# JakobHavtorn/benchmarking-lvms

Measured on AMD Instinct MI355X. Metric: audio frames/sec training (VRNN, 16 kHz mu-law), higher is better.
Workload: dtype f32

## Files before the change

benchmarking-lvms_amd/blvm/_hip.py:

```python
import ctypes
import os

import torch

_LIB_PATH = os.environ.get("BLVM_HIP_LIB") or os.path.join(os.path.dirname(os.path.abspath(__file__)), "lib", "libblvm_hip.so")
_lib = None

c_int, c_float, c_void_p, c_size_t, c_double = ctypes.c_int, ctypes.c_float, ctypes.c_void_p, ctypes.c_size_t, ctypes.c_double


class BlvmHipError(RuntimeError):
    pass


class VrnnWeights(ctypes.Structure):

    _fields_ = [
        ("prior_w", c_void_p * 3), ("prior_b", c_void_p * 3), ("prior_hw", c_void_p), ("prior_hb", c_void_p),
        ("post_w", c_void_p * 3), ("post_b", c_void_p * 3), ("post_hw", c_void_p), ("post_hb", c_void_p),
        ("phi_w", c_void_p * 4), ("phi_b", c_void_p * 4),
        ("gru_wih", c_void_p), ("gru_whh", c_void_p), ("gru_bih", c_void_p), ("gru_bhh", c_void_p),
    ]


class VrnnDecodeWeights(ctypes.Structure):

    _fields_ = [
        ("enc_w", c_void_p * 3), ("enc_b", c_void_p * 3), ("cell", ctypes.POINTER(VrnnWeights)),
        ("dec_w", c_void_p * 3), ("dec_b", c_void_p * 3), ("lik_w", c_void_p), ("lik_b", c_void_p),
    ]


class SrnnWeights(ctypes.Structure):

    _fields_ = [
        ("prior_w", c_void_p * 3), ("prior_b", c_void_p * 3), ("prior_hw", c_void_p), ("prior_hb", c_void_p),
        ("post_w", c_void_p * 3), ("post_b", c_void_p * 3), ("post_hw", c_void_p), ("post_hb", c_void_p),
    ]


class SrnnDecodeWeights(ctypes.Structure):

    _fields_ = [
        ("enc_w", c_void_p * 3), ("enc_b", c_void_p * 3), ("gru_wih", c_void_p), ("gru_whh", c_void_p), ("gru_bih", c_void_p),
        ("gru_bhh", c_void_p), ("chain", ctypes.POINTER(SrnnWeights)), ("dec_w", c_void_p * 3), ("dec_b", c_void_p * 3),
        ("lik_w", c_void_p), ("lik_b", c_void_p),
    ]


class LstmDecodeWeights(ctypes.Structure):

    _fields_ = [
        ("emb_w", c_void_p * 3), ("emb_b", c_void_p * 3), ("wih", ctypes.POINTER(c_void_p)), ("whh", ctypes.POINTER(c_void_p)),
        ("bih", ctypes.POINTER(c_void_p)), ("bhh", ctypes.POINTER(c_void_p)), ("dec_w", c_void_p * 3), ("dec_b", c_void_p * 3),
        ("lik_w", c_void_p), ("lik_b", c_void_p),
    ]


class RssmWeights(ctypes.Structure):

    _fields_ = [
        ("gin_w", c_void_p), ("gin_b", c_void_p), ("gru_wih", c_void_p), ("gru_whh", c_void_p), ("gru_bih", c_void_p),
        ("gru_bhh", c_void_p),
        ("prior_w", c_void_p * 3), ("prior_b", c_void_p * 3), ("prior_hw", c_void_p), ("prior_hb", c_void_p),
        ("post_w", c_void_p * 3), ("post_b", c_void_p * 3), ("post_hw", c_void_p), ("post_hb", c_void_p),
    ]


_SIGNATURES = {
    "blvm_upload_i32": (c_int, [c_void_p, c_int, c_void_p, c_void_p]),
    "blvm_version": (c_int, []),
    "blvm_last_error": (ctypes.c_char_p, []),
    "blvm_device_ok": (c_int, []),
    "blvm_async_errors": (c_int, [c_void_p]),
    "blvm_async_errors_take": (c_int, [c_void_p]),
    "blvm_pchain_configure": (c_int, [c_int, c_int]),
    "blvm_pchain_max_batch": (c_int, []),
    "blvm_set_operand_dtype": (c_int, [c_int]),
    "blvm_get_operand_dtype": (c_int, []),
    "blvm_pchain_profile": (c_int, [c_void_p]),
    "blvm_pchain_tune": (c_int, [c_int]),
    "blvm_pchain_static": (c_int, [c_int]),
    "blvm_rnn_path_counts": (c_int, [c_void_p]),
    "blvm_rssm_path_counts": (c_int, [c_void_p]),
    "blvm_pchain_chain_probe": (c_int, [c_void_p, c_void_p, c_void_p, c_void_p, c_int, c_int, c_int, c_int, c_void_p]),
    "blvm_pchain_static_chain_probe": (c_int, [c_void_p, c_void_p, c_void_p, c_void_p, c_int, c_int, c_int, c_int, c_void_p]),
    "blvm_pchain_static_chain_probe_fetch": (c_int, [c_void_p, c_void_p, c_void_p, c_void_p, c_int, c_int, c_int, c_int, c_void_p]),
    "blvm_pchain_static_chain_probe_paced": (c_int, [c_void_p, c_void_p, c_void_p, c_void_p] + [c_int] * 6 + [c_void_p]),
    "blvm_pchain_rows_to_t16": (c_int, [c_void_p, c_int, c_int, c_int, c_void_p, c_void_p]),
    "blvm_gemm_f32": (c_int, [c_int, c_int, c_int, c_int, c_int, c_void_p, c_int, c_void_p, c_int, c_void_p, c_int,
                              c_void_p, c_int, c_float, c_void_p, c_int, c_int, c_int, c_void_p]),
    "blvm_act_bwd_f32": (c_int, [c_void_p, c_void_p, c_float, c_void_p, c_size_t, c_void_p]),
    "blvm_colsum_f32": (c_int, [c_int, c_int, c_void_p, c_int, c_void_p, c_int, c_void_p]),
    "blvm_wgrad_f32": (c_int, [c_int, c_int, c_int, c_void_p, c_int, c_void_p, c_int, c_void_p, c_int, c_void_p, c_int, c_void_p]),
    "blvm_wgrad_group_f32": (c_int, [c_int, c_void_p, c_void_p, c_int, c_void_p, c_void_p, c_void_p, c_void_p, c_void_p, c_void_p, c_void_p, c_void_p]),
    "blvm_dmol_fwd": (c_int, [c_void_p, c_int, c_void_p, c_void_p, c_void_p, c_void_p, c_int, c_int, c_int, c_int,
                              c_int, c_int, c_float, c_void_p, c_void_p, c_void_p]),
    "blvm_dmol_bwd": (c_int, [c_void_p, c_int, c_void_p, c_void_p, c_void_p, c_void_p, c_void_p, c_int, c_int, c_int,
                              c_int, c_int, c_int, c_float, c_void_p, c_void_p, c_void_p]),
    "blvm_dmol_bwd_fused_workspace_floats": (c_size_t, [c_int] * 3),
    "blvm_dmol_bwd_fused": (c_int, [c_void_p, c_int, c_void_p, c_void_p, c_void_p, c_void_p, c_void_p, c_int, c_int, c_int,
                                    c_int, c_int, c_int, c_float, c_float, c_void_p, c_void_p, c_void_p, c_void_p, c_void_p]),
    "blvm_elbo_fwd": (c_int, [c_void_p, c_void_p, c_void_p, c_double, c_double, c_int, c_int, c_void_p, c_void_p, c_void_p, c_void_p]),
    "blvm_elbo_bwd": (c_int, [c_void_p, c_void_p, c_double, c_double, c_int, c_void_p, c_void_p, c_void_p]),
    "blvm_kl_fwd": (c_int, [c_void_p, c_void_p, c_void_p, c_void_p, c_int, c_void_p, c_int, c_int, c_int, c_int,
                            c_float, c_void_p, c_void_p, c_void_p]),
    "blvm_kl_bwd": (c_int, [c_void_p, c_void_p, c_void_p, c_void_p, c_int, c_void_p, c_void_p, c_void_p, c_int, c_int,
                            c_int, c_int, c_float, c_void_p, c_void_p, c_void_p, c_void_p, c_void_p]),
    "blvm_vrnn_decode_scratch_floats": (c_size_t, [c_int] * 4),
    "blvm_vrnn_decode": (c_int, [ctypes.POINTER(VrnnDecodeWeights)] + [c_void_p] * 5 + [c_int] * 7 + [c_float] * 3 + [c_void_p] * 4),
    "blvm_srnn_generate_scratch_floats": (c_size_t, [c_int] * 6),
    "blvm_srnn_generate": (c_int, [ctypes.POINTER(SrnnDecodeWeights)] + [c_void_p] * 6 + [c_int] * 7 + [c_float] * 3 + [c_void_p] * 5),
    "blvm_lstm_generate_scratch_floats": (c_size_t, [c_int] * 5),
    "blvm_lstm_generate": (c_int, [ctypes.POINTER(LstmDecodeWeights)] + [c_void_p] * 5 + [c_int] * 6 + [c_float] + [c_void_p] * 5),
    "blvm_lstm_generate_any_stack": (c_int, [ctypes.POINTER(LstmDecodeWeights)] + [c_void_p] * 5 + [c_int] * 6 + [c_float] + [c_void_p] * 5),
    "blvm_vrnn_generate_scratch_floats": (c_size_t, [c_int] * 6),
    "blvm_vrnn_generate": (c_int, [ctypes.POINTER(VrnnDecodeWeights)] + [c_void_p] * 5 + [c_int] * 7 + [c_float] * 3 + [c_void_p] * 4),
    "blvm_vrnn_reserve_floats": (c_size_t, [c_int] * 6),
    "blvm_vrnn_bwd_workspace_floats": (c_size_t, [c_int] * 6),
    "blvm_vrnn_seq_fwd": (c_int, [ctypes.POINTER(VrnnWeights), c_void_p, c_void_p, c_void_p, c_int, c_int, c_int, c_int,
                                  c_int, c_int, c_int, c_float, c_void_p, c_void_p, c_void_p, c_void_p, c_void_p,
                                  c_void_p, c_void_p, c_void_p]),
    "blvm_vrnn_seq_bwd": (c_int, [ctypes.POINTER(VrnnWeights), c_void_p, c_void_p, c_void_p, c_void_p, c_void_p,
                                  c_void_p, c_void_p, c_void_p, c_void_p, c_void_p, c_void_p, c_void_p, c_void_p,
                                  c_int, c_float, c_int, c_int, c_int, c_int, c_int, c_int, c_int, c_float, c_void_p,
                                  c_void_p, ctypes.POINTER(VrnnWeights), c_void_p, c_void_p]),
    "blvm_lstm_reserve_floats": (c_size_t, [c_int] * 3),
    "blvm_lstm_bwd_workspace_floats": (c_size_t, [c_int] * 3),
    "blvm_lstm_seq_fwd": (c_int, [c_void_p] * 8 + [c_int] * 4 + [c_void_p] * 5),
    "blvm_lstm_seq_bwd": (c_int, [c_void_p] * 5 + [c_int] * 4 + [c_void_p] * 9),
    "blvm_gru_reserve_floats": (c_size_t, [c_int] * 3),
    "blvm_gru_bwd_workspace_floats": (c_size_t, [c_int] * 3),
    "blvm_gru_seq_fwd": (c_int, [c_void_p] * 5 + [c_int, c_void_p, c_void_p] + [c_int] * 5 + [c_void_p, ctypes.c_longlong, c_int]
                         + [c_void_p] * 3),
    "blvm_gru_seq_bwd": (c_int, [c_void_p] * 3 + [c_int, c_void_p, c_int, c_void_p, c_void_p, ctypes.c_longlong, c_int]
                         + [c_int] * 4 + [c_void_p, c_int, c_int] + [c_void_p] * 7),
    "blvm_srnn_reserve_floats": (c_size_t, [c_int] * 5),
    "blvm_srnn_bwd_workspace_floats": (c_size_t, [c_int] * 5),
    "blvm_srnn_latent_fwd": (c_int, [ctypes.POINTER(SrnnWeights)] + [c_void_p] * 4 + [c_int] * 6 + [c_float, c_float]
                             + [c_void_p] * 7),
    "blvm_srnn_latent_bwd": (c_int, [ctypes.POINTER(SrnnWeights)] + [c_void_p] * 13 + [c_int, c_float] + [c_int] * 6
                             + [c_float, c_float] + [c_void_p] * 3 + [ctypes.POINTER(SrnnWeights), c_void_p, c_void_p]),
    "blvm_scale_act_f32": (c_int, [c_void_p, c_float, c_float, c_void_p, c_size_t, c_void_p]),
    "blvm_conv1d_k2_workspace_floats": (c_size_t, [c_int] * 2),
    "blvm_conv1d_k2_fwd": (c_int, [c_void_p] * 3 + [c_int] * 5 + [c_void_p] * 3),
    "blvm_conv1d_k2_bwd": (c_int, [c_void_p] * 3 + [c_int] * 5 + [c_void_p] * 5),
    "blvm_wavenet_block_reserve_floats": (c_size_t, [c_int] * 4),
    "blvm_wavenet_block_workspace_floats": (c_size_t, [c_int] * 5),
    "blvm_wavenet_block_fwd": (c_int, [c_void_p] * 5 + [c_int] * 6 + [c_float] + [c_void_p] * 5),
    "blvm_wavenet_block_bwd": (c_int, [c_void_p] * 6 + [c_int] * 6 + [c_float] + [c_void_p] * 7),
    "blvm_wavenet_stack_floats": (c_int, [c_int] * 3 + [c_void_p, c_int, c_void_p, c_void_p]),
    "blvm_wavenet_stack_fwd": (c_int, [c_void_p] * 4 + [c_int] * 6 + [c_float] + [c_void_p] * 5),
    "blvm_wavenet_stack_bwd": (c_int, [c_void_p] * 4 + [c_int] * 6 + [c_float] + [c_void_p] * 8),
    "blvm_wavenet_decode_pack_floats": (c_size_t, [c_int] * 4),
    "blvm_wavenet_decode_scratch_floats": (c_size_t, [c_void_p] + [c_int] * 4),
    "blvm_wavenet_decode": (c_int, [c_void_p] * 2 + [c_int] * 7 + [c_float] * 3 + [c_void_p] * 5),
    "blvm_wavenet_decode_ring_offset_floats": (c_size_t, [c_int] * 3),
    "blvm_wavenet_decode_ring_fill": (c_int, [c_void_p] + [c_int] * 5 + [c_void_p] * 2),
    "blvm_wavenet_decode_resume": (c_int, [c_void_p] * 2 + [c_int] * 8 + [c_float] * 3 + [c_void_p] * 7),
    "blvm_stcn_generate_pack_floats": (c_size_t, [c_int] * 4 + [c_void_p] * 2 + [c_int] * 3),
    "blvm_stcn_generate_scratch_floats": (c_size_t, [c_void_p] + [c_int] * 4 + [c_void_p] * 2 + [c_int] * 4),
    "blvm_stcn_generate": (c_int, [c_void_p] * 3 + [c_int] * 2 + [c_void_p] * 2 + [c_int] * 7 + [c_float] * 6 + [c_void_p] * 9),
    "blvm_stcn_generate_ring_offset_floats": (c_size_t, [c_int] * 4 + [c_void_p] * 2 + [c_int] * 3),
    "blvm_stcn_generate_resume": (c_int, [c_void_p] * 3 + [c_int] * 2 + [c_void_p] * 2 + [c_int] * 7 + [c_float] * 6 + [c_void_p] * 8
                                  + [c_int] + [c_void_p] * 3),
    "blvm_rssm_reserve_floats": (c_size_t, [c_int] * 4),
    "blvm_rssm_bwd_workspace_floats": (c_size_t, [c_int] * 4),
    "blvm_rssm_seq_fwd": (c_int, [ctypes.POINTER(RssmWeights)] + [c_void_p] * 5 + [c_int] * 7 + [c_float] + [c_void_p] * 8),
    "blvm_rssm_seq_bwd": (c_int, [ctypes.POINTER(RssmWeights)] + [c_void_p] * 15 + [c_int, c_float] + [c_int] * 7 + [c_float]
                          + [c_void_p] * 4 + [ctypes.POINTER(RssmWeights), c_void_p, c_void_p]),
    "blvm_gmm_fwd": (c_int, [c_void_p, c_int] + [c_void_p] * 4 + [c_int] * 5 + [c_float] * 2 + [c_void_p] * 3),
    "blvm_gmm_bwd": (c_int, [c_void_p, c_int] + [c_void_p] * 5 + [c_int] * 5 + [c_float] * 2 + [c_void_p] * 3),
    "blvm_gauss_head_fwd": (c_int, [c_void_p, c_int] + [c_void_p] * 4 + [c_int] * 4 + [c_float] * 2 + [c_void_p] * 3),
    "blvm_gauss_head_bwd": (c_int, [c_void_p, c_int] + [c_void_p] * 5 + [c_int] * 4 + [c_float] * 2 + [c_void_p] * 3),
# ... 112 lines not shown
```

benchmarking-lvms_amd/csrc/common.h:

```cpp
#pragma once
#include <hip/hip_runtime.h>
#include <limits.h>
#include <stdint.h>
#include <stdio.h>

#include "blvm_hip.h"

namespace blvm {

typedef float f32x4 __attribute__((ext_vector_type(4)));
typedef float f32x16 __attribute__((ext_vector_type(16)));

void set_error(const char* fmt, ...);

#define BLVM_REQUIRE(cond, ...)            \
  do {                                     \
    if (!(cond)) {                         \
      blvm::set_error(__VA_ARGS__);        \
      return BLVM_EINVAL;                  \
    }                                      \
  } while (0)

#define BLVM_CHECK_LAUNCH(what)                                                     \
  do {                                                                              \
// ... 210 lines not shown
}

template <int NW, bool WT16 = false>
__device__ __forceinline__ f32x16 wave_gemm32(const float* __restrict__ A, int lda, int r0, int nrows,
                                               const float* __restrict__ W, int ldw, int c0, int K, int wave, f32x16 acc) {
  constexpr int STEP = NW * 8;
  const int lane = threadIdx.x & 63, li = lane & 31, lh = lane >> 5;
  const bool aok = (r0 + li) < nrows;
  const float* ap = A + (size_t)(aok ? r0 + li : 0) * lda + 4 * lh;
  const float* wp = WT16 ? W + (size_t)(c0 / 16 + (li >> 4)) * ldw * 16 + ((li & 15) + 16 * lh) * 4 : W + (size_t)(c0 + li) * ldw + 4 * lh;
  constexpr int WS = WT16 ? 16 : 1;
  const float4 zero = make_float4(0.f, 0.f, 0.f, 0.f);
  int kc = wave * 8;
  for (; kc + 3 * STEP < K; kc += 4 * STEP) {
    float4 a0 = *reinterpret_cast<const float4*>(ap + kc);
    float4 a1 = *reinterpret_cast<const float4*>(ap + kc + STEP);
    float4 a2 = *reinterpret_cast<const float4*>(ap + kc + 2 * STEP);
    float4 a3 = *reinterpret_cast<const float4*>(ap + kc + 3 * STEP);
    const float4 w0 = *reinterpret_cast<const float4*>(wp + WS * (kc));
    const float4 w1 = *reinterpret_cast<const float4*>(wp + WS * (kc + STEP));
    const float4 w2 = *reinterpret_cast<const float4*>(wp + WS * (kc + 2 * STEP));
    const float4 w3 = *reinterpret_cast<const float4*>(wp + WS * (kc + 3 * STEP));
    if (!aok) { a0 = a1 = a2 = a3 = zero; }
    acc = __builtin_amdgcn_mfma_f32_32x32x2f32(a0.x, w0.x, acc, 0, 0, 0);
    acc = __builtin_amdgcn_mfma_f32_32x32x2f32(a0.y, w0.y, acc, 0, 0, 0);
    acc = __builtin_amdgcn_mfma_f32_32x32x2f32(a0.z, w0.z, acc, 0, 0, 0);
    acc = __builtin_amdgcn_mfma_f32_32x32x2f32(a0.w, w0.w, acc, 0, 0, 0);
    acc = __builtin_amdgcn_mfma_f32_32x32x2f32(a1.x, w1.x, acc, 0, 0, 0);
    acc = __builtin_amdgcn_mfma_f32_32x32x2f32(a1.y, w1.y, acc, 0, 0, 0);
    acc = __builtin_amdgcn_mfma_f32_32x32x2f32(a1.z, w1.z, acc, 0, 0, 0);
    acc = __builtin_amdgcn_mfma_f32_32x32x2f32(a1.w, w1.w, acc, 0, 0, 0);
    acc = __builtin_amdgcn_mfma_f32_32x32x2f32(a2.x, w2.x, acc, 0, 0, 0);
    acc = __builtin_amdgcn_mfma_f32_32x32x2f32(a2.y, w2.y, acc, 0, 0, 0);
    acc = __builtin_amdgcn_mfma_f32_32x32x2f32(a2.z, w2.z, acc, 0, 0, 0);
    acc = __builtin_amdgcn_mfma_f32_32x32x2f32(a2.w, w2.w, acc, 0, 0, 0);
    acc = __builtin_amdgcn_mfma_f32_32x32x2f32(a3.x, w3.x, acc, 0, 0, 0);
    acc = __builtin_amdgcn_mfma_f32_32x32x2f32(a3.y, w3.y, acc, 0, 0, 0);
    acc = __builtin_amdgcn_mfma_f32_32x32x2f32(a3.z, w3.z, acc, 0, 0, 0);
    acc = __builtin_amdgcn_mfma_f32_32x32x2f32(a3.w, w3.w, acc, 0, 0, 0);
  }
  for (; kc < K; kc += STEP) {
    float4 a0 = *reinterpret_cast<const float4*>(ap + kc);
    const float4 w0 = *reinterpret_cast<const float4*>(wp + WS * (kc));
    if (!aok) a0 = zero;
    acc = __builtin_amdgcn_mfma_f32_32x32x2f32(a0.x, w0.x, acc, 0, 0, 0);
    acc = __builtin_amdgcn_mfma_f32_32x32x2f32(a0.y, w0.y, acc, 0, 0, 0);
    acc = __builtin_amdgcn_mfma_f32_32x32x2f32(a0.z, w0.z, acc, 0, 0, 0);
    acc = __builtin_amdgcn_mfma_f32_32x32x2f32(a0.w, w0.w, acc, 0, 0, 0);
  }
  return acc;
}

template <int G, int NW>
__device__ __forceinline__ void reduce_tiles(const f32x4 (&acc)[G], float* __restrict__ red, float (&out)[G]) {
  const int tid = threadIdx.x, lane = tid & 63, wave = tid >> 6;
#pragma unroll
  for (int g = 0; g < G; ++g) {
#pragma unroll
    for (int r = 0; r < 4; ++r) red[(g * NW + wave) * 256 + ((lane >> 4) * 4 + r) * 16 + (lane & 15)] = acc[g][r];
  }
  __syncthreads();
#pragma unroll
  for (int g = 0; g < G; ++g) {
    float s = 0.f;
    if (tid < 256) {
#pragma unroll
      for (int w = 0; w < NW; ++w) s += red[(g * NW + w) * 256 + tid];
    }
    out[g] = s;
  }
}

}

namespace blvm {
int pchain_ctl(unsigned** dev, unsigned** host_dev, unsigned* epoch);
int pchain_max_batch();
int pchain_tune();
unsigned long long* pchain_profile_buffer();

int gemm_f32(int op_a, int op_b, int M, int N, int K, const float* A, int lda, const float* B, int ldb, float* C,
             int ldc, const float* bias, int act, float slope, const float* gate, int ldg, int accumulate,
             int split_k, hipStream_t stream, float* colsum = nullptr);
int colsum_f32(int M, int N, const float* X, int ldx, float* out, int accumulate, hipStream_t stream);
struct WgradJob {
  const float* D; int ldd, M;
  const float* Act; int lda, N;
  float* dW; int ldw;
  float* db;
};
int gemm_wgrad_group(const WgradJob* jobs, int njobs, int K, hipStream_t stream);
int transpose_f32(int M, int N, const float* X, int ldx, float* out, int ldo, hipStream_t stream);
enum OpType { OP_F32 = 0, OP_BF16 = 1, OP_F16 = 2 };
OpType operand_type();
inline bool operand_16bit() { return operand_type() != OP_F32; }
struct T16PackScope {
  T16PackScope(OpType ot, hipStream_t stream);
  ~T16PackScope();
  int flush();
  T16PackScope(const T16PackScope&) = delete;
  T16PackScope& operator=(const T16PackScope&) = delete;
 private:
  OpType prev_;
  bool prev_active_;
};
int t16_pack(const float* src, long rs, long cs, int R, int K, float* dst, hipStream_t stream);
inline int t16_pack_rows(const float* W, int ldw, int R, int K, float* dst, hipStream_t s) { return t16_pack(W, ldw, 1, R, K, dst, s); }
inline int t16_pack_transposed(const float* X, int ldx, int M, int N, float* dst, hipStream_t s) { return t16_pack(X, 1, ldx, N, M, dst, s); }

}
```

benchmarking-lvms_amd/csrc/gemm.hip:

```cpp
#include <algorithm>
#include <type_traits>

#include <vector>

#include "common.h"

namespace blvm {

namespace {

constexpr int BK = 16;
constexpr int BK64 = 32;
constexpr int tile_bk(int bm, int bn) { return (bm == 64 && bn == 64) ? BK64 : BK; }

constexpr int PAD = 4;
constexpr int PAD_T = 2;

struct GemmArgs {
  const float* A;
  const float* B;
  float* C;
  const float* bias;
  const float* gate;
  int M, N, K, lda, ldb, ldc, ldg;
// ... 521 lines not shown
  }
}

__global__ __launch_bounds__(256) void act_bwd_kernel(const float* dy, const float* y, float slope, float* dz, size_t n4,
                                                      size_t n) {
  for (size_t i = (size_t)blockIdx.x * 256 + threadIdx.x; i < n4; i += (size_t)gridDim.x * 256) {
    const float4 g = reinterpret_cast<const float4*>(dy)[i];
    const float4 v = reinterpret_cast<const float4*>(y)[i];
    float4 o;
    o.x = v.x > 0.f ? g.x : g.x * slope;
    o.y = v.y > 0.f ? g.y : g.y * slope;
    o.z = v.z > 0.f ? g.z : g.z * slope;
    o.w = v.w > 0.f ? g.w : g.w * slope;
    reinterpret_cast<float4*>(dz)[i] = o;
  }
  if (blockIdx.x == 0) {
    const size_t i = n4 * 4 + threadIdx.x;
    if (i < n) dz[i] = y[i] > 0.f ? dy[i] : dy[i] * slope;
  }
}

__global__ __launch_bounds__(256) void transpose_kernel(int M, int N, const float* __restrict__ X, int ldx,
                                                        float* __restrict__ out, int ldo) {
  __shared__ float t[32][33];
  const int tx = threadIdx.x & 31, ty = threadIdx.x >> 5;
  const int m0 = blockIdx.y * 32, n0 = blockIdx.x * 32;
  for (int i = ty; i < 32; i += 8)
    if (m0 + i < M && n0 + tx < N) t[i][tx] = X[(size_t)(m0 + i) * ldx + n0 + tx];
  __syncthreads();
  for (int i = ty; i < 32; i += 8)
    if (n0 + i < N && m0 + tx < M) out[(size_t)(n0 + i) * ldo + m0 + tx] = t[tx][i];
}

bool wgrad_fits(const float* D, int ldd, int M, const float* Act, int lda, int N, int K) {
  return aligned16(D) && aligned16(Act) && ldd % 4 == 0 && lda % 4 == 0 && M % 4 == 0 && N % 4 == 0 && K >= 1024;
}
int wgrad_tiles(int M, int N) { return ((M + WBM - 1) / WBM) * ((N + WBM - 1) / WBM); }
int wgrad_split(long tiles, int K) {
  static const int cus = [] {
    int dev = 0, n = 0;
    if (hipGetDevice(&dev) != hipSuccess || hipDeviceGetAttribute(&n, hipDeviceAttributeMultiprocessorCount, dev) != hipSuccess) n = 0;
    return n > 0 ? n : 256;
  }();
  long split = (160 / (WST * 16)) * (long)cus / std::max(1L, tiles);
  split = std::min<long>(split, K / (32 * WBK));
  return (int)std::max(1L, split);
}
int wgrad_k_per_split(int K, int split) {
  const int ksteps = (K + WBK - 1) / WBK;
  return ((ksteps + split - 1) / split) * WBK;
}

}

int gemm_f32(int op_a, int op_b, int M, int N, int K, const float* A, int lda, const float* B, int ldb, float* C,
             int ldc, const float* bias, int act, float slope, const float* gate, int ldg, int accumulate,
             int split_k, hipStream_t stream, float* colsum) {
  BLVM_REQUIRE(M >= 0 && N >= 0 && K >= 0, "gemm: negative dimension");
  if (M == 0 || N == 0) return BLVM_OK;
  BLVM_REQUIRE(A && B && C, "gemm: null operand");
  BLVM_REQUIRE(act >= 0 && act <= 2, "gemm: unknown activation %d", act);
  BLVM_REQUIRE(lda >= (op_a ? M : K) && ldb >= (op_b ? N : K) && ldc >= N, "gemm: leading dimension too small");
  GemmArgs g;
  g.A = A; g.B = B; g.C = C; g.bias = bias; g.gate = gate;
  g.M = M; g.N = N; g.K = K; g.lda = lda; g.ldb = ldb; g.ldc = ldc; g.ldg = ldg;
  g.act = act; g.slope = slope; g.accumulate = accumulate;
  g.a_vec = aligned16(A) && (lda % 4 == 0);
  g.b_vec = aligned16(B) && (ldb % 4 == 0);
  if (split_k < 1) split_k = 1;
  const bool wgrad_wins = (long)M * N >= 512L * 512 || (K >= 32768 && std::max(M, N) >= 256);
  if (op_a == 1 && op_b == 1 && operand_type() == OP_F32 && act == 0 && gate == nullptr && bias == nullptr && wgrad_wins &&
      wgrad_fits(A, lda, M, B, ldb, N, K)) {
    g.colsum = colsum;
    const int split = split_k == 1 ? 1 : wgrad_split(wgrad_tiles(M, N), K);
    g.k_per_split = wgrad_k_per_split(K, split);
    const int nz = (K + g.k_per_split - 1) / g.k_per_split;
    const dim3 grid((N + WBM - 1) / WBM, (M + WBM - 1) / WBM, nz);
    if (nz > 1 && !accumulate)
      BLVM_HIP(hipMemset2DAsync(C, sizeof(float) * (size_t)ldc, 0, sizeof(float) * (size_t)N, (size_t)M, stream));
    hipLaunchKernelGGL(wgrad_kernel, grid, dim3(256), 0, stream, g);
    BLVM_CHECK_LAUNCH("gemm_f32");
    return BLVM_OK;
  }
  bool big =(M >= 128 && N >= 128 && (size_t)((M + 127) / 128) * ((N + 127) / 128) * split_k >= 192);
  static const int force_tile = [] { const char* e = getenv("BLVM_GEMM_TILE"); return e ? atoi(e) : 0; }();
  if ((op_a == 1 && op_b == 1) || (K <= 256 && N <= 256)) big = false;
  if (force_tile == 1) big = false;
  const bool n192 = big && N % 192 == 0 && N % 128 != 0 && force_tile != 2;
  const bool m192 = big && !n192 && M % 192 == 0 && M % 128 != 0;
  const int bm = big ? (m192 ? 192 : 128) : 64;
  const int bn = big ? (n192 ? 192 : 128) : 64;
  const OpType ot = operand_type();
  const int bk = ot != OP_F32 ? BKB : tile_bk(bm, bn);
  if (colsum != nullptr && (ot != OP_F32 || op_a != 1 || K == 0)) {
    BLVM_TRY(op_a == 1 ? colsum_f32(K, M, A, lda, colsum, 1, stream) : BLVM_EINVAL);
    colsum = nullptr;
  }
  g.colsum = colsum;
  int ksteps = (K + bk - 1) / bk;
  if (split_k > ksteps) split_k = ksteps > 0 ? ksteps : 1;
  g.k_per_split = ((ksteps + split_k - 1) / split_k) * bk;
  if (g.k_per_split == 0) g.k_per_split = bk;
  split_k = (K + g.k_per_split - 1) / g.k_per_split;
  if (split_k < 1) split_k = 1;
  BLVM_REQUIRE(split_k == 1 || (act == 0 && gate == nullptr), "gemm: split-K needs a linear epilogue");
  dim3 grid((N + bn - 1) / bn, (M + bm - 1) / bm, split_k);
  BLVM_REQUIRE(grid.y <= 65535 && grid.z <= 65535, "gemm: grid too large");
  if (split_k > 1 && !accumulate)
    BLVM_HIP(hipMemset2DAsync(C, sizeof(float) * (size_t)ldc, 0, sizeof(float) * (size_t)N, (size_t)M, stream));
  if (n192) launch_gemm<128, 192>(g, op_a, op_b, grid, stream, ot);
  else if (m192) launch_gemm<192, 128>(g, op_a, op_b, grid, stream, ot);
  else if (big) launch_gemm<128, 128>(g, op_a, op_b, grid, stream, ot);
  else launch_gemm<64, 64>(g, op_a, op_b, grid, stream, ot);
  BLVM_CHECK_LAUNCH("gemm_f32");
  return BLVM_OK;
}

int gemm_wgrad_group(const WgradJob* jobs, int njobs, int K, hipStream_t stream) {
  std::vector<int> take;
  for (int i = 0; i < njobs; ++i) {
    const WgradJob& j = jobs[i];
    if (!j.dW) {
      if (j.db) BLVM_TRY(colsum_f32(K, j.M, j.D, j.ldd, j.db, 1, stream));
      continue;
    }
    BLVM_REQUIRE(j.D && j.Act && j.M > 0 && j.N > 0 && j.ldd >= j.M && j.lda >= j.N && j.ldw >= j.N, "gemm_wgrad_group: bad job %d", i);
    if (!operand_16bit() && wgrad_fits(j.D, j.ldd, j.M, j.Act, j.lda, j.N, K) && (int)take.size() < kMaxGroup) {
      take.push_back(i);
      continue;
    }
    BLVM_TRY(gemm_f32(1, 1, j.M, j.N, K, j.D, j.ldd, j.Act, j.lda, j.dW, j.ldw, nullptr, 0, 0.f, nullptr, 0, 1, gemm_pick_split(j.M, j.N, K), stream, j.db));
  }
  if (take.size() < 2) {
    for (const int i : take) {
      const WgradJob& j = jobs[i];
      BLVM_TRY(gemm_f32(1, 1, j.M, j.N, K, j.D, j.ldd, j.Act, j.lda, j.dW, j.ldw, nullptr, 0, 0.f, nullptr, 0, 1, gemm_pick_split(j.M, j.N, K), stream, j.db));
    }
    return BLVM_OK;
  }
  std::stable_sort(take.begin(), take.end(), [&](int x, int y) { return (long)jobs[x].M * jobs[x].N > (long)jobs[y].M * jobs[y].N; });
  GemmGroup gg;
  gg.n = 0;
  long tiles = 0;
  for (const int i : take) {
    const WgradJob& j = jobs[i];
    GemmArgs& g = gg.p[gg.n++];
    g = GemmArgs{};
    g.A = j.D; g.B = j.Act; g.C = j.dW;
    g.M = j.M; g.N = j.N; g.K = K; g.lda = j.ldd; g.ldb = j.lda; g.ldc = j.ldw;
    g.accumulate = 1;
    g.colsum = j.db;
    tiles += wgrad_tiles(j.M, j.N);
  }
  long area = 0;
  for (int p = 0; p < gg.n; ++p) area += (long)gg.p[p].M * gg.p[p].N;
  const bool dma = area * 100 >= tiles * WBM * WBM * 95L;
  const int bk = dma ? WBK : tile_bk(64, 64);
  int split;
  if (dma) {
    split = wgrad_split(tiles, K);
  } else {
    long tiles64 = 0;
    for (int p = 0; p < gg.n; ++p) tiles64 += (long)((gg.p[p].M + 63) / 64) * ((gg.p[p].N + 63) / 64);
    split = (int)std::max(1L, std::min<long>((1536 + tiles64 - 1) / tiles64, (K + bk - 1) / bk / 16));
  }
  const int ksteps = (K + bk - 1) / bk;
  const int k_per_split = ((ksteps + split - 1) / split) * bk;
  gg.split = (K + k_per_split - 1) / k_per_split;
// ... 224 lines not shown
```

include/blvm_hip.h:

```cpp
#ifndef BLVM_HIP_H
#define BLVM_HIP_H

#include <stddef.h>
#include <stdint.h>

#ifdef __cplusplus
extern "C" {
#endif

#define BLVM_OK 0
#define BLVM_EINVAL (-1)
#define BLVM_ELAUNCH (-2)
#define BLVM_ENOSUP (-3)
#define BLVM_NOT_APPLICABLE 1

int blvm_version(void);
const char* blvm_last_error(void);
int blvm_device_ok(void);
int blvm_async_errors(unsigned* last_code);
int blvm_async_errors_take(unsigned* last_code);
int blvm_pchain_configure(int max_batch, int waves);
int blvm_pchain_max_batch(void);
#define BLVM_DTYPE_F32 0
#define BLVM_DTYPE_BF16 1
#define BLVM_DTYPE_F16 2
int blvm_set_operand_dtype(int dtype);
int blvm_get_operand_dtype(void);
int blvm_pchain_profile(unsigned long long* device_buffer);
int blvm_pchain_tune(int bits);
int blvm_pchain_static(int mode);
int blvm_rnn_path_counts(unsigned long long out[12]);
int blvm_rssm_path_counts(unsigned long long out[6]);
int blvm_pchain_chain_probe(const float* W16, const float* bias, float* x16, float* xs, int B, int N, int L, int nwg, void* stream);
int blvm_pchain_static_chain_probe(const float* W16, const float* bias, float* x16, float* xs, int B, int N, int L, int nwg, void* stream);
int blvm_pchain_static_chain_probe_fetch(const float* W16, const float* bias, float* x16, float* xs, int B, int N, int L, int nwg, void* stream);
int blvm_pchain_static_chain_probe_paced(const float* W16, const float* bias, float* x16, float* xs, int B, int N, int L, int nwg,
                                         int early_delay, int epi_delay, void* stream);
int blvm_pchain_rows_to_t16(const float* src, int ld, int B, int K, float* dst, void* stream);
int blvm_upload_i32(const int32_t* host, int n, int32_t* dst, void* stream);

int blvm_gemm_f32(int op_a, int op_b, int M, int N, int K, const float* A, int lda, const float* B, int ldb,
                  float* C, int ldc, const float* bias, int act, float slope, const float* gate, int ldg,
                  int accumulate, int split_k, void* stream);

int blvm_act_bwd_f32(const float* dy, const float* y, float slope, float* dz, size_t n, void* stream);

int blvm_wgrad_f32(int N_out, int K_in, int rows, const float* D, int ldd, const float* X, int ldx, float* dW, int lddw, float* db,
                   int split_k, void* stream);

int blvm_wgrad_group_f32(int n, const int* N_out, const int* K_in, int rows, const float* const* D, const int* ldd, const float* const* X,
                         const int* ldx, float* const* dW, const int* lddw, float* const* db, void* stream);

int blvm_colsum_f32(int M, int N, const float* X, int ldx, float* out, int accumulate, void* stream);

int blvm_dmol_fwd(const float* dec, int layout, const float* W, const float* bias, const float* y,
                  const int32_t* x_sl, int B, int T, int Tp, int S, int num_mix, int num_bins, float log_eps,
                  double* log_prob, float* ll_twise, void* stream);

int blvm_dmol_bwd(const float* dec, int layout, const float* W, const float* bias, const float* y,
                  const int32_t* x_sl, const float* g_b, int B, int T, int Tp, int S, int num_mix, int num_bins,
                  float log_eps, float* d_dec, float* d_par, void* stream);

size_t blvm_dmol_bwd_fused_workspace_floats(int B, int Tp, int S);
int blvm_dmol_bwd_fused(const float* dec, int layout, const float* W, const float* bias, const float* y,
                        const int32_t* x_sl, const float* g_b, int B, int T, int Tp, int S, int num_mix, int num_bins,
                        float log_eps, float act_slope, float* dz, float* dW, float* db, float* workspace, void* stream);

int blvm_gmm_fwd(const float* dec, int layout, const float* W, const float* bias, const float* y, const int32_t* x_sl,
                 int B, int T, int Tp, int S, int num_mix, float sd_beta, float sd_eps, double* log_prob, float* ll_twise,
                 void* stream);
int blvm_gmm_bwd(const float* dec, int layout, const float* W, const float* bias, const float* y, const int32_t* x_sl,
                 const float* g_b, int B, int T, int Tp, int S, int num_mix, float sd_beta, float sd_eps, float* d_dec,
                 float* d_par, void* stream);
int blvm_gauss_head_fwd(const float* dec, int layout, const float* W, const float* bias, const float* y,
                        const int32_t* x_sl, int B, int T, int Tp, int S, float sd_beta, float sd_eps, double* log_prob,
                        float* ll_twise, void* stream);
int blvm_gauss_head_bwd(const float* dec, int layout, const float* W, const float* bias, const float* y,
                        const int32_t* x_sl, const float* g_b, int B, int T, int Tp, int S, float sd_beta, float sd_eps,
                        float* d_dec, float* d_par, void* stream);

int blvm_mix_sample(const float* par, const float* u, const float* v, long long n, int num_mix, int kind, float log_eps,
                    float sd_beta, float sd_eps, float* out, void* stream);

int blvm_kl_fwd(const float* mu_q, const float* sd_q, const float* mu_p, const float* sd_p, int layout,
                const int32_t* x_sl, int B, int Tp, int Z, int stride, float fn_floor, double* kld,
                double* kld_fn, void* stream);

int blvm_kl_bwd(const float* mu_q, const float* sd_q, const float* mu_p, const float* sd_p, int layout,
                const int32_t* x_sl, const float* c_raw, const float* c_fn, int B, int Tp, int Z, int stride,
                float fn_floor, float* d_mu_q, float* d_sd_q, float* d_mu_p, float* d_sd_p, void* stream);

int blvm_elbo_fwd(const double* log_prob, const double* kld, const double* kld_fn, double beta, double n_frames, int B,
                  int kl_raw, double* elbo, double* loss, double* sums, void* stream);
int blvm_elbo_bwd(const double* g_loss, const double* g_elbo, double beta, double n_frames, int B, double* g64, float* g32,
                  void* stream);

int blvm_gauss_latent_fwd(const float* mu_p, const float* sd_p_raw, const float* mu_q_raw, const float* sd_q_raw,
                          const float* eps, size_t n, float beta_p, float beta_q, float sd_eps, int mode, float* sd_p,
                          float* mu_q, float* sd_q, float* z, void* stream);
int blvm_gauss_latent_bwd(const float* mu_p, const float* sd_p_raw, const float* mu_q_raw, const float* sd_q_raw,
                          const float* eps, const float* g_sd_p, const float* g_mu_q, const float* g_sd_q, const float* g_z,
                          size_t n, float beta_p, float beta_q, float sd_eps, int mode, float* d_mu_p, float* d_sd_p_raw,
                          float* d_mu_q_raw, float* d_sd_q_raw, void* stream);

typedef struct BlvmVrnnWeights {
  const float *prior_w[3], *prior_b[3];
  const float *prior_hw, *prior_hb;
  const float *post_w[3], *post_b[3];
  const float *post_hw, *post_hb;
  const float *phi_w[4], *phi_b[4];
  const float *gru_wih, *gru_whh;
  const float *gru_bih, *gru_bhh;
} BlvmVrnnWeights;

typedef struct BlvmVrnnGrads {
  float *prior_w[3], *prior_b[3], *prior_hw, *prior_hb;
  float *post_w[3], *post_b[3], *post_hw, *post_hb;
  float *phi_w[4], *phi_b[4];
  float *gru_wih, *gru_whh, *gru_bih, *gru_bhh;
} BlvmVrnnGrads;

typedef struct BlvmVrnnDecodeWeights {
  const float *enc_w[3], *enc_b[3];
  const BlvmVrnnWeights* cell;
  const float *dec_w[3], *dec_b[3];
  const float *lik_w, *lik_b;
} BlvmVrnnDecodeWeights;
// ... 211 lines not shown
```

Baseline: 87.78 million.

## Add weight-stationary MFMA GEMM path for tall, small-K f32 GEMMs

Adds a new weight-stationary GEMM kernel that keeps each wave's 16-column slab of B in registers and streams A row-blocks through double-buffered LDS, using f32 MFMA 16x16x4. It is used for non-transposed A with K<=256, K and N multiples of 16, and M>=256. Rows are split into ranges across CUs, which targets the many tall-skinny layer GEMMs in the VRNN MLPs that the generic tiled kernel handles poorly. The change also adds routing and path-count APIs and moves the env tile override ahead of the new route. The risk is lower efficiency than the existing path for some shapes, and a reliance on permlane swap instructions.

Result: faster. 88.80 million (median of 6 runs) (+1.2%).

```diff
diff --git a/benchmarking-lvms_amd/blvm/_hip.py b/benchmarking-lvms_amd/blvm/_hip.py
--- a/benchmarking-lvms_amd/blvm/_hip.py
+++ b/benchmarking-lvms_amd/blvm/_hip.py
@@ -90,6 +90,9 @@
     "blvm_pchain_rows_to_t16": (c_int, [c_void_p, c_int, c_int, c_int, c_void_p, c_void_p]),
     "blvm_gemm_f32": (c_int, [c_int, c_int, c_int, c_int, c_int, c_void_p, c_int, c_void_p, c_int, c_void_p, c_int,
                               c_void_p, c_int, c_float, c_void_p, c_int, c_int, c_int, c_void_p]),
+    "blvm_gemm_ws_route": (c_int, [c_int, c_int, c_int, c_int, c_size_t, c_int, c_int, c_int, c_int, c_int]),
+    "blvm_gemm_ws_min_rows": (c_int, [c_int]),
+    "blvm_gemm_path_counts": (c_int, [c_void_p]),
     "blvm_act_bwd_f32": (c_int, [c_void_p, c_void_p, c_float, c_void_p, c_size_t, c_void_p]),
     "blvm_colsum_f32": (c_int, [c_int, c_int, c_void_p, c_int, c_void_p, c_int, c_void_p]),
     "blvm_wgrad_f32": (c_int, [c_int, c_int, c_int, c_void_p, c_int, c_void_p, c_int, c_void_p, c_int, c_void_p, c_int, c_void_p]),
diff --git a/benchmarking-lvms_amd/csrc/common.h b/benchmarking-lvms_amd/csrc/common.h
--- a/benchmarking-lvms_amd/csrc/common.h
+++ b/benchmarking-lvms_amd/csrc/common.h
@@ -316,6 +316,11 @@
 int gemm_f32(int op_a, int op_b, int M, int N, int K, const float* A, int lda, const float* B, int ldb, float* C,
              int ldc, const float* bias, int act, float slope, const float* gate, int ldg, int accumulate,
              int split_k, hipStream_t stream, float* colsum = nullptr);
+bool gemm_ws_route(int op_a, int M, int N, int K, uintptr_t a_addr, int lda, int split_k, bool has_colsum, int operand, int min_rows);
+int gemm_ws_min_rows();
+int gemm_ws_f32(int op_b, int M, int N, int K, const float* A, int lda, const float* B, int ldb, float* C, int ldc, const float* bias,
+                int act, float slope, const float* gate, int ldg, int accumulate, hipStream_t stream);
+void gemm_count_path(int path);
 int colsum_f32(int M, int N, const float* X, int ldx, float* out, int accumulate, hipStream_t stream);
 struct WgradJob {
   const float* D; int ldd, M;
diff --git a/benchmarking-lvms_amd/csrc/gemm.hip b/benchmarking-lvms_amd/csrc/gemm.hip
--- a/benchmarking-lvms_amd/csrc/gemm.hip
+++ b/benchmarking-lvms_amd/csrc/gemm.hip
@@ -627,8 +627,14 @@
     BLVM_CHECK_LAUNCH("gemm_f32");
     return BLVM_OK;
   }
+  static const int force_tile = [] { const char* e = getenv("BLVM_GEMM_TILE"); return e ? atoi(e) : 0; }();
+  if (force_tile != 3 && gemm_ws_route(op_a, M, N, K, reinterpret_cast<uintptr_t>(A), lda, split_k, colsum != nullptr, operand_type(),
+                                       gemm_ws_min_rows())) {
+    gemm_count_path(1);
+    return gemm_ws_f32(op_b, M, N, K, A, lda, B, ldb, C, ldc, bias, act, slope, gate, ldg, accumulate, stream);
+  }
+  gemm_count_path(0);
   bool big =(M >= 128 && N >= 128 && (size_t)((M + 127) / 128) * ((N + 127) / 128) * split_k >= 192);
-  static const int force_tile = [] { const char* e = getenv("BLVM_GEMM_TILE"); return e ? atoi(e) : 0; }();
   if ((op_a == 1 && op_b == 1) || (K <= 256 && N <= 256)) big = false;
   if (force_tile == 1) big = false;
   const bool n192 = big && N % 192 == 0 && N % 128 != 0 && force_tile != 2;
diff --git a/benchmarking-lvms_amd/csrc/gemm_ws.hip b/benchmarking-lvms_amd/csrc/gemm_ws.hip
--- /dev/null
+++ b/benchmarking-lvms_amd/csrc/gemm_ws.hip
@@ -0,0 +1,264 @@
+#include <atomic>
+
+#include "common.h"
+
+namespace blvm {
+
+namespace {
+
+constexpr int WS_WAVES = 8;
+constexpr int WS_RB = 2;
+constexpr int WS_THREADS = WS_WAVES * 64;
+
+struct WsArgs {
+  const float* A;
+  const float* B;
+  float* C;
+  const float* bias;
+  const float* gate;
+  int M, N, lda, ldb, ldc, ldg;
+  int act;
+  float slope;
+  int accumulate;
+  int ncg, nranges, stages_per_range;
+  int b_vec, c_vec, g_vec;
+};
+
+__device__ __forceinline__ void lane_swap16(float& a, float& b) {
+  asm volatile("s_nop 1\n\tv_permlane16_swap_b32 %0, %1" : "+v"(a), "+v"(b));
+}
+__device__ __forceinline__ void lane_swap32(float& a, float& b) {
+  asm volatile("s_nop 1\n\tv_permlane32_swap_b32 %0, %1" : "+v"(a), "+v"(b));
+}
+
+template <int NC, int OPB>
+__global__ __launch_bounds__(WS_THREADS) __attribute__((amdgpu_waves_per_eu(2, 2))) void gemm_ws_kernel(WsArgs g) {
+  constexpr int K = 16 * NC, S = K + 8, ROWS = 16 * WS_RB;
+  constexpr int ITEMS = ROWS * (K / 4);
+  constexpr int NV = (ITEMS + WS_THREADS - 1) / WS_THREADS;
+  __shared__ __attribute__((aligned(16))) float lds[2][ROWS * S];
+
+  const int tid = threadIdx.x, lane = tid & 63, i = lane & 15, q = lane >> 4;
+  const int wave = __builtin_amdgcn_readfirstlane(tid >> 6);
+  const int cg = blockIdx.x % g.ncg, range = blockIdx.x / g.ncg;
+  const int slab = cg * WS_WAVES + wave;
+  const bool active = slab * 16 < g.N;
+  const int n0 = slab * 16;
+
+  const int nblocks = (g.M + 15) >> 4, nstages = (nblocks + WS_RB - 1) / WS_RB;
+  const int s0 = range * g.stages_per_range, s1 = min(nstages, s0 + g.stages_per_range);
+
+  f32x4 r[NV];
+  auto gload = [&](int st) {
+#pragma unroll
+    for (int v = 0; v < NV; ++v) {
+      const int id = tid + v * WS_THREADS;
+      if (ITEMS % WS_THREADS == 0 || id < ITEMS) {
+        const int row = id / (K / 4), c4 = id % (K / 4);
+        r[v] = *reinterpret_cast<const f32x4*>(g.A + (size_t)min(st * ROWS + row, g.M - 1) * g.lda + 4 * c4);
+      }
+    }
+  };
+  auto swrite = [&](float* dst) {
+#pragma unroll
+    for (int v = 0; v < NV; ++v) {
+      const int id = tid + v * WS_THREADS;
+      if (ITEMS % WS_THREADS == 0 || id < ITEMS) {
+        const int j = id % (K / 4);
+        float* d = dst + (id / (K / 4)) * S + 16 * (j >> 2) + (j & 3);
+#pragma unroll
+        for (int x = 0; x < 4; ++x) d[4 * x] = r[v][x];
+      }
+    }
+  };
+
+  gload(s0);
+
+  f32x4 w[NC];
+  f32x4 bv = {0.f, 0.f, 0.f, 0.f};
+  const int nq = n0 + 4 * q;
+  if (active) {
+    if (OPB == 0 && g.b_vec) {
+      const float* wp = g.B + (size_t)(n0 + i) * g.ldb + 4 * q;
+#pragma unroll
+      for (int c = 0; c < NC; ++c) {
+        const f32x4 t = *reinterpret_cast<const f32x4*>(wp + 16 * c);
+        float t0 = t[0], t1 = t[1], t2 = t[2], t3 = t[3];
+        lane_swap16(t0, t1);
+        lane_swap16(t2, t3);
+        lane_swap32(t0, t2);
+        lane_swap32(t1, t3);
+        w[c] = f32x4{t0, t1, t2, t3};
+      }
+    } else {
+      const float* wp = OPB == 0 ? g.B + (size_t)(n0 + i) * g.ldb + q : g.B + (size_t)q * g.ldb + n0 + i;
+      const size_t ks = OPB == 0 ? 1 : (size_t)g.ldb;
+#pragma unroll
+      for (int c = 0; c < NC; ++c)
+#pragma unroll
+        for (int e = 0; e < 4; ++e) w[c][e] = wp[(size_t)(16 * c + 4 * e) * ks];
+    }
+    if (g.bias != nullptr) {
+#pragma unroll
+      for (int e = 0; e < 4; ++e) bv[e] = g.bias[nq + e];
+    }
+  } else {
+#pragma unroll
+    for (int c = 0; c < NC; ++c) w[c] = bv;
+  }
+
+  auto lds_read = [&](f32x4 (&a)[NC], const float* src) {
+    const float* ap = src + i * S + 4 * q;
+#pragma unroll
+    for (int c = 0; c < NC; ++c) a[c] = *reinterpret_cast<const f32x4*>(ap + 16 * c);
+  };
+  auto epilogue = [&](f32x4 v, f32x4 gt, f32x4 cv, float* cp, bool ok) {
+    v += bv;
+    if (g.act == 1) {
+#pragma unroll
+      for (int e = 0; e < 4; ++e) v[e] = v[e] > 0.f ? v[e] : 0.f;
+    } else if (g.act == 2) {
+#pragma unroll
+      for (int e = 0; e < 4; ++e) v[e] = v[e] > 0.f ? v[e] : v[e] * g.slope;
+    }
+    if (g.gate != nullptr) {
+#pragma unroll
+      for (int e = 0; e < 4; ++e) v[e] *= gt[e] > 0.f ? 1.f : g.slope;
+    }
+    if (g.accumulate) v += cv;
+    if (!ok) return;
+    if (g.c_vec) *reinterpret_cast<f32x4*>(cp) = v;
+    else {
+#pragma unroll
+      for (int e = 0; e < 4; ++e) cp[e] = v[e];
+    }
+  };
+
+  swrite(lds[0]);
+  __syncthreads();
+  for (int st = s0; st < s1; ++st) {
+    const float* cur = lds[(st - s0) & 1];
+    float* nxt = lds[((st - s0) & 1) ^ 1];
+    gload(min(st + 1, nstages - 1));
+    if (active) {
+      f32x4 gt[WS_RB], cv[WS_RB], a[WS_RB][NC], acc[WS_RB];
+      float* cp[WS_RB];
+      bool ok[WS_RB];
+#pragma unroll
+      for (int s = 0; s < WS_RB; ++s) {
+        const int m = (st * WS_RB + s) * 16 + i;
+        ok[s] = m < g.M;
+        cp[s] = g.C + (size_t)(ok[s] ? m : 0) * g.ldc + nq;
+        gt[s] = cv[s] = bv;
+        if (g.gate != nullptr && ok[s]) {
+          const float* gp = g.gate + (size_t)m * g.ldg + nq;
+          if (g.g_vec) gt[s] = *reinterpret_cast<const f32x4*>(gp);
+          else {
+#pragma unroll
+            for (int e = 0; e < 4; ++e) gt[s][e] = gp[e];
+          }
+        }
+        if (g.accumulate && ok[s]) {
+          if (g.c_vec) cv[s] = *reinterpret_cast<const f32x4*>(cp[s]);
+          else {
+#pragma unroll
+            for (int e = 0; e < 4; ++e) cv[s][e] = cp[s][e];
+          }
+        }
+      }
+#pragma unroll
+      for (int s = 0; s < WS_RB; ++s) {
+        lds_read(a[s], cur + s * 16 * S);
+        acc[s] = f32x4{0.f, 0.f, 0.f, 0.f};
+      }
+      __builtin_amdgcn_sched_barrier(0);
+#pragma unroll
+      for (int c = 0; c < NC; ++c)
+#pragma unroll
+        for (int e = 0; e < 4; ++e)
+#pragma unroll
+          for (int s = 0; s < WS_RB; ++s) acc[s] = __builtin_amdgcn_mfma_f32_16x16x4f32(w[c][e], a[s][c][e], acc[s], 0, 0, 0);
+      __builtin_amdgcn_sched_barrier(0);
+      swrite(nxt);
+#pragma unroll
+      for (int s = 0; s < WS_RB; ++s) epilogue(acc[s], gt[s], cv[s], cp[s], ok[s]);
+    } else {
+      swrite(nxt);
+    }
+    __syncthreads();
+  }
+}
+
+std::atomic<unsigned long long> g_path_count[2];
+constexpr int kWsMinRowsDefault = 256;
+std::atomic<int> g_ws_min_rows{kWsMinRowsDefault};
+
+int cu_count() {
+  static const int cus = [] {
+    int dev = 0, n = 0;
+    if (hipGetDevice(&dev) != hipSuccess || hipDeviceGetAttribute(&n, hipDeviceAttributeMultiprocessorCount, dev) != hipSuccess) n = 0;
+    return n > 0 ? n : 256;
+  }();
+  return cus;
+}
+
+template <int OPB>
+void launch_ws(int nc, const WsArgs& g, dim3 grid, hipStream_t s) {
+#define WS_CASE(n) case n: hipLaunchKernelGGL((gemm_ws_kernel<n, OPB>), grid, dim3(WS_THREADS), 0, s, g); break;
+  switch (nc) {
+    WS_CASE(1) WS_CASE(2) WS_CASE(3) WS_CASE(4) WS_CASE(5) WS_CASE(6) WS_CASE(7) WS_CASE(8)
+    WS_CASE(9) WS_CASE(10) WS_CASE(11) WS_CASE(12) WS_CASE(13) WS_CASE(14) WS_CASE(15) WS_CASE(16)
+  }
+#undef WS_CASE
+}
+
+}
+
+void gemm_count_path(int path) { g_path_count[path != 0].fetch_add(1, std::memory_order_relaxed); }
+int gemm_ws_min_rows() { return g_ws_min_rows.load(std::memory_order_relaxed); }
+
+bool gemm_ws_route(int op_a, int M, int N, int K, uintptr_t a_addr, int lda, int split_k, bool has_colsum, int operand, int min_rows) {
+  return operand == OP_F32 && op_a == 0 && split_k == 1 && !has_colsum && K > 0 && K % 16 == 0 && K <= 256 && N > 0 && N % 16 == 0 &&
+         (a_addr & 15u) == 0 && lda % 4 == 0 && M >= min_rows && M >= 1;
+}
+
+int gemm_ws_f32(int op_b, int M, int N, int K, const float* A, int lda, const float* B, int ldb, float* C, int ldc, const float* bias,
+                int act, float slope, const float* gate, int ldg, int accumulate, hipStream_t stream) {
+  BLVM_REQUIRE(M <= INT_MAX - 16 * WS_RB, "gemm: too many rows");
+  WsArgs g;
+  g.A = A; g.B = B; g.C = C; g.bias = bias; g.gate = gate;
+  g.M = M; g.N = N; g.lda = lda; g.ldb = ldb; g.ldc = ldc; g.ldg = ldg;
+  g.act = act; g.slope = slope; g.accumulate = accumulate;
+  g.b_vec = aligned16(B) && ldb % 4 == 0;
+  g.c_vec = aligned16(C) && ldc % 4 == 0;
+  g.g_vec = gate != nullptr && aligned16(gate) && ldg % 4 == 0;
+  const int nstages = ((M + 15) / 16 + WS_RB - 1) / WS_RB;
+  g.ncg = (N / 16 + WS_WAVES - 1) / WS_WAVES;
+  const long nranges = std::max(1L, std::min<long>(nstages, cu_count() / g.ncg));
+  g.stages_per_range = (int)((nstages + nranges - 1) / nranges);
+  g.nranges = (nstages + g.stages_per_range - 1) / g.stages_per_range;
+  const long groups = (long)g.ncg * g.nranges;
+  BLVM_REQUIRE(groups < (1L << 31) - 1, "gemm: grid too large");
+  const dim3 grid((unsigned)groups);
+  if (op_b == 0) launch_ws<0>(K / 16, g, grid, stream);
+  else launch_ws<1>(K / 16, g, grid, stream);
+  BLVM_CHECK_LAUNCH("gemm_f32");
+  return BLVM_OK;
+}
+
+}
+
+extern "C" int blvm_gemm_path_counts(unsigned long long* out) {
+  BLVM_REQUIRE(out != nullptr, "blvm_gemm_path_counts: null pointer");
+  for (int p = 0; p < 2; ++p) out[p] = blvm::g_path_count[p].load(std::memory_order_relaxed);
+  return BLVM_OK;
+}
+
+extern "C" int blvm_gemm_ws_min_rows(int rows) {
+  return blvm::g_ws_min_rows.exchange(rows < 0 ? blvm::kWsMinRowsDefault : rows, std::memory_order_relaxed);
+}
+
+extern "C" int blvm_gemm_ws_route(int op_a, int M, int N, int K, size_t a_addr, int lda, int split_k, int has_colsum, int operand,
+                                  int min_rows) {
+  return blvm::gemm_ws_route(op_a, M, N, K, (uintptr_t)a_addr, lda, split_k, has_colsum != 0, operand, min_rows) ? 1 : 0;
+}
diff --git a/include/blvm_hip.h b/include/blvm_hip.h
--- a/include/blvm_hip.h
+++ b/include/blvm_hip.h
@@ -43,6 +43,10 @@
                   float* C, int ldc, const float* bias, int act, float slope, const float* gate, int ldg,
                   int accumulate, int split_k, void* stream);
 
+int blvm_gemm_ws_route(int op_a, int M, int N, int K, size_t a_addr, int lda, int split_k, int has_colsum, int operand, int min_rows);
+int blvm_gemm_ws_min_rows(int rows);
+int blvm_gemm_path_counts(unsigned long long* out);
+
 int blvm_act_bwd_f32(const float* dy, const float* y, float slope, float* dz, size_t n, void* stream);
 
 int blvm_wgrad_f32(int N_out, int K_in, int rows, const float* D, int ldd, const float* X, int ldx, float* dW, int lddw, float* db,
```
